# mspaintenjoyer/DepthEstimation

Hardware: AMD Instinct MI355X
Metric: disparity Mpix/s at 1080p d_max=128; 1/2/4/8-GPU scaling + %HBM roofline (higher is better)
Workload: dtype u8

## Files before the change

depthestimation_amd/csrc/dsx_api.hip:

```cpp
#include <hip/hip_runtime.h>

#include <cstdio>
#include <cstdlib>
#include <algorithm>
#include <cstring>
#include <string>
#include <vector>

#include "../../include/dsx.h"
#include "dsx_internal.h"

extern char **environ;

#ifndef DSX_RESET_LEFT
#define DSX_RESET_LEFT 1
#endif

namespace {

thread_local std::string g_err;

int fail(int code, const std::string &msg) {
    g_err = msg;
    return code;
// ... 365 lines not shown
        take("PRIO_T", e.prio_t);
        take("SLOW_W8", e.slow_w8);
        take("AGEW", e.agew);
        take("VARIANT", e.variant);
        take("TIMELINE", e.timeline);
    }
    return e;
}

dsx::Bm2Args base_args(dsx_handle *h, int H, int W, int64_t stride, const DsxEnv &env = dsx_env()) {
    dsx::Bm2Args a{};
    a.stride = stride;
    a.H = H;
    a.W = W;
    a.m = h->p.min_disp;
    a.D = h->p.num_disp;
    a.uniq = h->p.uniqueness_ratio;
    a.lr = h->p.disp12_max_diff;
    a.subpix = h->p.subpixel;
    a.float_mode = h->p.float_mode;
    a.padv = pad_value(h);
    a.strip_begin = 0;
    a.strip_count = (W + dsx::kStripWidth - 1) / dsx::kStripWidth;
    a.grid_override = h->p.grid_blocks;
    {
        const bool fl = h->p.in_flight != 0;
        a.prio = env.prio ? atoi(env.prio) : (fl ? 0 : 1);
        a.pt1 = 128, a.pt2 = 205, a.pt3 = 243;
        if (env.prio_t) sscanf(env.prio_t, "%d,%d,%d", &a.pt1, &a.pt2, &a.pt3);
        a.slow_w8 = env.slow_w8 ? atoi(env.slow_w8) : 11;
        a.agew[0] = fl ? 64 : 78, a.agew[1] = fl ? 64 : 70, a.agew[2] = a.agew[3] = 64;
        if (env.agew) sscanf(env.agew, "%d,%d,%d,%d", &a.agew[0], &a.agew[1], &a.agew[2], &a.agew[3]);
        a.nlev = 0;
        a.variant = env.variant ? atoi(env.variant) : 0;
    }
    a.nframes = 1;
    a.frame_stride = 0;
    return a;
}

#define DSX_LAUNCH(h, name, st, call)                                    \
    do {                                                                 \
        TimedLaunch t_;                                                  \
        if ((h)->p.timing) {                                             \
            int rc_ = begin_timed((h), (name), (st), t_);                \
            if (rc_) return rc_;                                         \
// ... 70 lines not shown
        a.ref = static_cast<const uint8_t *>(dL);
        a.src = static_cast<const uint8_t *>(dR);
        a.out_fixed = static_cast<int16_t *>(outFixed);
        a.out_float = static_cast<float *>(outFloat);
        a.nframes = nframes;
        a.frame_stride = frame_stride;
        if (lr) {
            a.side = dsx::SIDE_LEFT_LR;
            a.lr_keys = h->lrKeys + (size_t)h->lrParity * H * W * h->lrFrames;
            a.lr_reset = h->lrKeys + (size_t)(h->lrParity ^ 1) * H * W * h->lrFrames;
            a.lr_reset_n = DSX_RESET_LEFT ? (int64_t)H * W * h->lrDirty[h->lrParity ^ 1] : 0;
            a.dstar = h->dStar;
            a.kshift = h->g.kind != dsx::BM_SAD ? h->g.DB : 16;
        } else {
            if (lr_sg) {
                a.sg_keys = h->lrKeys + (size_t)h->lrParity * H * W * h->lrFrames;
                a.lr_reset = h->lrKeys + (size_t)(h->lrParity ^ 1) * H * W * h->lrFrames;
                a.lr_reset_n = (int64_t)H * W * h->lrDirty[h->lrParity ^ 1];
                a.dstar = h->dStar;
                a.kshift = h->g.kind != dsx::BM_SAD ? h->g.DB : 16;
            }
            const int xlo = std::max(0, h->p.min_disp + h->p.num_disp - 1);
            const int xhi = std::min(W - 1, W - 1 + h->p.min_disp);
            if (xlo > xhi) {
                a.strip_begin = 0;
                a.strip_count = 0;
            } else {
                a.strip_begin = xlo / dsx::kStripWidth;
                a.strip_count = xhi / dsx::kStripWidth + 1 - a.strip_begin;
            }
        }
        uint64_t *tl = nullptr;
        const char *tlpath = env.timeline;
        if (tlpath && *tlpath) DSX_HIP(hipMalloc(&tl, 12 * 8 * 65536));
        if (tl) DSX_HIP(hipMemsetAsync(tl, 0, 12 * 8 * 65536, st));
        a.timeline = tl;
        DSX_LAUNCH(h, "bm_pass_left", st, dsx::launch_bm2(radius, h->g.kind, h->g.NW, a, st));
        h->lastKeys = lr_sg ? a.sg_keys : (lr ? a.lr_keys : nullptr);
        h->lastDstar = h->dStar;
        h->lastKshift = a.kshift;
        if (lr_sg) {
            const int P = h->lrParity;
            if (!defer_lr)
                DSX_LAUNCH(h, "lr_fixup_sgbm", st,
                           dsx::launch_lr_fixup_sgbm(h->dStar, a.sg_keys, H * nframes, W, h->p.min_disp,
                                                     h->p.disp12_max_diff, a.kshift, a.out_fixed, a.out_float, st));
            h->lrDirty[P ^ 1] = 0;
            h->lrDirty[P] = nframes;
            h->lrParity = P ^ 1;
// ... 763 lines not shown
```

depthestimation_amd/csrc/dsx_bm.hip:

```cpp
#include "dsx_internal.h"
#include "dsx_partition.h"
#include "dsx_subpix.h"

constexpr int kWpe = 3;
constexpr int kWpeSsd = 4;

#ifndef DSX_ROWSTEP_PAIRTAIL
#define DSX_ROWSTEP_PAIRTAIL 0
#endif
#ifndef DSX_ROWSTEP_DIVQ
#define DSX_ROWSTEP_DIVQ 1
#endif
#ifndef DSX_ROWSTEP_OVERLAP
#define DSX_ROWSTEP_OVERLAP 1
#endif
#ifndef DSX_ROWSTEP_AHEAD
#define DSX_ROWSTEP_AHEAD 1
#endif
constexpr bool kRowstepOverlap = DSX_ROWSTEP_OVERLAP;
constexpr bool kRowstepAhead = DSX_ROWSTEP_AHEAD;
constexpr bool kRowstepPairtail = DSX_ROWSTEP_PAIRTAIL;
constexpr bool kRowstepDivq = DSX_ROWSTEP_DIVQ;
#ifndef DSX_ROWSTEP_ATID
#define DSX_ROWSTEP_ATID 1
#endif
#ifndef DSX_ROWSTEP_KEY2
#define DSX_ROWSTEP_KEY2 1
#endif
#ifndef DSX_ROWSTEP_MERGE
#define DSX_ROWSTEP_MERGE 1
#endif
constexpr bool kRowstepMerge = DSX_ROWSTEP_MERGE;
constexpr bool kRowstepAtid = DSX_ROWSTEP_ATID;
constexpr bool kRowstepKey2 = DSX_ROWSTEP_KEY2;

#include <algorithm>
#include <cstdio>
#include <cstdlib>
#include <cstring>
#include <mutex>
#include <type_traits>
#include <utility>
#include <vector>

namespace dsx {

typedef unsigned short u16x2 __attribute__((ext_vector_type(2)));
typedef uint32_t u32x2 __attribute__((ext_vector_type(2)));
__device__ __forceinline__ u32x2 lds_read_b64(const uint8_t *p) {
    return *(const volatile __attribute__((address_space(3))) u32x2 *)p;
}

__device__ __forceinline__ u16x2 as2(uint32_t v) { return __builtin_bit_cast(u16x2, v); }
__device__ __forceinline__ uint32_t as1(u16x2 v) { return __builtin_bit_cast(uint32_t, v); }
__device__ __forceinline__ int clampi2(int v, int lo, int hi) { return v < lo ? lo : (v > hi ? hi : v); }
__device__ __forceinline__ uint32_t umin2(uint32_t a, uint32_t b) { return a < b ? a : b; }
__device__ __forceinline__ u16x2 add_sub2(u16x2 a, u16x2 p, u16x2 q) { return as2(as1(a) + as1(p) - as1(q)); }
// ... 99 lines not shown
    return v;
}


typedef const __attribute__((address_space(4))) uint32_t cu32;
typedef const __attribute__((address_space(1))) uint8_t gu8;
typedef const __attribute__((address_space(1))) uint32_t gu32;
typedef __attribute__((address_space(1))) uint8_t gw8;
typedef __attribute__((address_space(1))) int16_t g16;
typedef __attribute__((address_space(1))) float gf32;

template <bool RELOAD>
__device__ __forceinline__ Bm2Args kargs_row(const Bm2Args &a) {
    if constexpr (RELOAD) {
        typedef __attribute__((address_space(4))) const Bm2Args KArgs;
        KArgs *p = (KArgs *)__builtin_amdgcn_kernarg_segment_ptr();
        asm volatile("" : "+s"(p));
        return *(const Bm2Args *)p;
    } else {
        return a;
    }
}

template <int R, bool SSD, int NW, int SIDE, bool FAST, bool ABS, bool LRFULL>
__device__ __forceinline__ void bm2_segment(const Bm2Args &a_in, uint8_t *smem, int x0, int yb, int ye, long fin, long fout,
                                            bool lr_on, int done0, const int (&pe)[3], int &qcur, int wvu
#ifdef DSX_STAMPS
                                            , uint64_t (&ph)[8], uint64_t &t_prev, uint64_t &nsteps
#endif
) {
    using G = Geo<R, SSD, NW>;
    constexpr int TX = G::TX, NC = G::NC, Dp = G::Dp, NT = G::NT, TPP = G::TPP, DSL = G::DSL, CB = G::CB,
                  PITCH = G::PITCH, NJ = G::NJ, SLOT = G::SLOT, NB = G::NB, NJ4 = (NJ + 3) / 4;
    constexpr int side = SIDE;
    const Bm2Args a = kargs_row<SIDE == 3>(a_in);
    constexpr bool FSS = SSD && !ABS && R <= 5 && (SIDE == 0 || SIDE == 3 || SIDE == 4);
    constexpr bool SGK = SIDE == 4;
    constexpr uint32_t OFF = FSS ? 0x4B000000u : 0u;
    constexpr int CW = (!FSS && (SSD || SIDE == 3)) ? 4 : 8, NCH = (NC + CW - 1) / CW;
    typedef typename std::conditional<FSS, float, typename std::conditional<SSD, uint32_t, u16x2>::type>::type acc_t;
    uint8_t *tile = smem + 4 * SLOT;

    constexpr bool LANE_RB = SSD && !ABS && NW >= 4;
    int ln = 0;
    if constexpr (LANE_RB)
        asm volatile("v_mbcnt_lo_u32_b32 %0, -1, 0\n\tv_mbcnt_hi_u32_b32 %0, -1, %0" : "=v"(ln));
    else
        ln = (int)threadIdx.x & 63;
    const int tid = LANE_RB ? (wvu << 6) + ln : (int)threadIdx.x;
    const int wv = LANE_RB ? wvu : tid >> 6;
    const int H = a.H, W = a.W, m = a.m, D = a.D;
    const int64_t stride = a.stride;
    const int d0 = SSD ? (wv * 64 + ln) : (wv * 128 + 2 * ln);
    const uint32_t padv = a.padv;
    const int PB = side == 1 ? (x0 - R + m) : (x0 - R - m + NC - 1);
    const int sgn = side == 1 ? 1 : -1;

    constexpr int NC4 = (NC + 3) / 4;
    constexpr bool RL2 = !SSD;
    uint32_t ofs_r = (uint32_t)(x0 - R + 4 * min(tid, NC4 - 1));
    uint32_t ofs_s = side == 1 ? (uint32_t)(PB + 4 * min(tid, NJ4 - 1)) : (uint32_t)(PB - 4 * min(tid, NJ4 - 1) - 3);
    constexpr bool MRG = kRowstepMerge && RL2 && FAST && SIDE != 3 && SIDE != 2 && !(SIDE == 4 && R >= 7);
    static_assert(!MRG || NJ4 + NC4 <= NT, "merged staging: a lane per staged dword");
    const bool m_s = tid < NJ4;
    const int m_r = min(tid - NJ4, NC4 - 1);
    const uint8_t *m_base = m_s ? a.src + fin + ofs_s : a.ref + fin + (uint32_t)(x0 - R + 4 * m_r);
    const bool m_dn = m_s && side != 1;
    const uint32_t m_sel0 = m_dn ? 0x0C0C0C03u : 0x0C0C0C00u, m_sel1 = m_dn ? 0x0C0C0C02u : 0x0C0C0C01u,
                   m_sel2 = m_dn ? 0x0C0C0C01u : 0x0C0C0C02u, m_sel3 = m_dn ? 0x0C0C0C00u : 0x0C0C0C03u;
    const uint32_t m_lane = m_s ? (uint32_t)(16 * tid) : (uint32_t)(G::SROW + 16 * m_r);
    auto ldm = [&](int r, uint32_t &w) __attribute__((always_inline)) {
        const int yy = clampi2(r, 0, H - 1);
        long ro = (long)yy * stride;
        asm("" : "+s"(ro));
        w = *reinterpret_cast<const uint32_t *>(m_base + ro);
    };
    auto stm = [&](uint8_t *sp, uint32_t w) __attribute__((always_inline)) {
        if (tid < NJ4 + NC4)
            *reinterpret_cast<uint4 *>(sp) = make_uint4(__builtin_amdgcn_perm(0u, w, m_sel0), __builtin_amdgcn_perm(0u, w, m_sel1),
                                                        __builtin_amdgcn_perm(0u, w, m_sel2), __builtin_amdgcn_perm(0u, w, m_sel3));
    };
    auto ld = [&](int r, uint32_t &w0, uint32_t &w1, uint32_t &w2, uint32_t &w3, uint32_t &rf) __attribute__((always_inline)) {
        const int yy = clampi2(r, 0, H - 1);
        const uint8_t *srow_ = a.src + fin + (long)yy * stride;
        const uint8_t *rrow_ = a.ref + fin + (long)yy * stride;
        if constexpr (RL2) {
            asm("" : "+s"(srow_));
            asm("" : "+s"(rrow_));
        }
        typedef typename std::conditional<RL2, gu8, const uint8_t>::type row8;
        typedef typename std::conditional<RL2, gu32, const uint32_t>::type row32;
        typedef typename std::conditional<RL2, uint32_t, int>::type rix;
// ... 128 lines not shown
    };
    auto pair_e0 = [](const uint32_t(&sw)[CW + 1], int c) __attribute__((always_inline)) -> uint32_t {
        return side == 1 ? sw[c] : sw[c + 1];
    };
    auto pair_e1 = [](const uint32_t(&sw)[CW + 1], int c) __attribute__((always_inline)) -> uint32_t {
        return side == 1 ? sw[c + 1] : sw[c];
    };

    acc_t cs[NC];
#pragma unroll
    for (int c = 0; c < NC; ++c) cs[c] = acc_t(0);
    constexpr bool SADINIT = ABS || R != 4 || SIDE != 3;
    if constexpr ((!SSD || ABS) && side != 1 && SADINIT) {
        constexpr int NGR = (2 * R + 1 + 3) / 4;
        constexpr int TPG = rnd16(NJ4 * 32);
        constexpr int RG = rnd16(NC4 * 16);
        static_assert(NGR * (TPG + RG) <= G::SMEM, "transposed init rows must fit the block's LDS");
        block_sync<NW>();
        auto ldb = [&](int r, uint32_t &w, uint32_t &e, uint32_t &rf) __attribute__((always_inline)) {
            const int yy = clampi2(r, 0, H - 1);
            const uint8_t *srow = a.src + fin + (long)yy * stride;
            const uint8_t *rrow = a.ref + fin + (long)yy * stride;
            const int tj = min(tid, NJ4 - 1), tr = min(tid, NC4 - 1);
            if constexpr (FAST) {
                const uint8_t *pp = srow + PB - 4 * tj - 3;
                w = *reinterpret_cast<const uint32_t *>(pp);
                e = pp[-1];
                rf = *reinterpret_cast<const uint32_t *>(rrow + x0 - R + 4 * tr);
            } else {
                uint32_t v = 0;
#pragma unroll
                for (int q = 0; q < 4; ++q) v |= (uint32_t)srow[clampi2(PB - 4 * tj - q, 0, W - 1)] << (8 * (3 - q));
                w = v;
                e = srow[clampi2(PB - 4 * tj - 4, 0, W - 1)];
                v = 0;
#pragma unroll
                for (int q = 0; q < 4; ++q) v |= (uint32_t)rrow[clampi2(x0 - R + 4 * tr + q, 0, W - 1)] << (8 * q);
                rf = v;
            }
        };
#pragma unroll 1
        for (int g = 0; g < NGR; ++g) {
            uint32_t w[4], e[4], rf[4];
#pragma unroll
            for (int r = 0; r < 4; ++r) {
                if (4 * g + r <= 2 * R) {
                    ldb(yb - R + 4 * g + r, w[r], e[r], rf[r]);
// ... 23 lines not shown
            }
            if (tid < NC4) {
                uint32_t Rv[4];
#pragma unroll
                for (int k = 0; k < 4; ++k) {
                    const uint32_t lo = __builtin_amdgcn_perm(rf[1], rf[0], 0x0C0C0000u | ((4u + k) << 8) | (uint32_t)k);
                    const uint32_t hi = __builtin_amdgcn_perm(rf[3], rf[2], 0x0C0C0000u | ((4u + k) << 8) | (uint32_t)k);
                    Rv[k] = __builtin_amdgcn_perm(hi, lo, 0x05040100u);
                }
                *reinterpret_cast<uint4 *>(smem + NGR * TPG + g * RG + 16 * tid) = make_uint4(Rv[0], Rv[1], Rv[2], Rv[3]);
            }
        }
        block_sync<NW>();
        const uint8_t *tb = smem + d0 * 8;
        {
        uint32_t ae[NC], ao[NC];
#pragma unroll
        for (int c = 0; c < NC; ++c) ae[c] = ao[c] = 0;
#pragma unroll 1
        for (int g = 0; g < NGR; ++g) {
#pragma unroll
            for (int q = 0; q < NC4; ++q) {
                const int c0 = 4 * q;
                const uint4 rr = *reinterpret_cast<const uint4 *>(smem + NGR * TPG + g * RG + 4 * c0);
                const uint32_t rv[4] = {rr.x, rr.y, rr.z, rr.w};
#pragma unroll
                for (int c = 0; c < 4; ++c) {
                    if (c0 + c < NC) {
                        if constexpr (ABS) {
                            const uint32_t p0 = *reinterpret_cast<const uint32_t *>(tb + g * TPG + (NC - 1 - c0 - c) * 8);
                            ae[c0 + c] = __builtin_amdgcn_sad_u8(rv[c], p0, ae[c0 + c]);
                        } else {
                            const uint2 pr = *reinterpret_cast<const uint2 *>(tb + g * TPG + (NC - 1 - c0 - c) * 8);
                            ae[c0 + c] = __builtin_amdgcn_sad_u8(rv[c], pr.x, ae[c0 + c]);
                            ao[c0 + c] = __builtin_amdgcn_sad_u8(rv[c], pr.y, ao[c0 + c]);
                        }
                    }
                }
            }
        }
#pragma unroll
        for (int c = 0; c < NC; ++c) {
            if constexpr (ABS) cs[c] = ae[c];
            else cs[c] = as2(ae[c] | (ao[c] << 16));
        }
        }
// ... 124 lines not shown
                for (int i = 0; i < 8; ++i) {
                    const bool hit = rel >= 8 * i - 1 && rel <= 8 * i + 8;
                    nm = hit ? nm : umin2(nm, emin8(*reinterpret_cast<const uint4 *>(epx + 16 * i)));
                }
                const int ib0 = (rel - 1) >> 3, ib1 = (rel + 1) >> 3;
#pragma unroll
                for (int t = 0; t < 2; ++t) {
                    const int ib = t == 0 ? ib0 : ib1;
                    if (ib >= 0 && ib < 8 && (t == 0 || ib1 != ib0)) {
                        const uint4 v = *reinterpret_cast<const uint4 *>(epx + 16 * ib);
                        const uint32_t c8[8] = {v.x & 0xFFFFu, v.x >> 16, v.y & 0xFFFFu, v.y >> 16,
                                                v.z & 0xFFFFu, v.z >> 16, v.w & 0xFFFFu, v.w >> 16};
#pragma unroll
                        for (int e = 0; e < 8; ++e) {
                            const int dd = 8 * ib + e - rel;
                            nm = (dd > 1 || dd < -1) ? umin2(nm, c8[e]) : nm;
                        }
                    }
                }
                nm = gmin<TPP>(nm);
                const uint32_t real_max = padv < (1u << 24) ? padv : (1u << 24);
                if (nm < real_max && nm * (uint32_t)(100 - a.uniq) < ecb * 100u) valid = false;
            }
            if (eh == 0 && ex < W) {
                const long o = fout + (long)ey * W + ex;
                const int16_t fx = valid ? (int16_t)(m * 16 + ef) : (int16_t)((m - 1) * 16);
                if (a.out_fixed) a.out_fixed[o] = fx;
                if (a.out_float) {
                    if (a.float_mode == 0) {
                        a.out_float[o] = (float)fx * 0.0625f;
                    } else {
                        float pf = (float)(m + eb);
                        if (esp) pf = (float)(m + eb) + (float)((int32_t)ecm - (int32_t)ecp) / (float)(2 * eden);
                        a.out_float[o] = valid ? pf : (float)(m - 1);
                    }
                }
            }
        }
    };
    for (int y = yb; y < ye; ++y) {
        const Bm2Args &a = kargs_row<SIDE == 3>(a_in);
#ifdef DSX_STAMPS
        ++nsteps;
#endif
        DSX_STAMP(0);
        if (a.prio) {
            const int dn = done0 + (y - yb);
// ... 64 lines not shown
                        sn[t][c + 1] = pn.x; sn[t][c] = pn.y; nxn = pn.x;
                        so[t][c + 1] = po.x; so[t][c] = po.y; nxo = po.x;
                    }
                }
            };
            auto sads = [&](auto qc) __attribute__((always_inline)) {
                constexpr int q = decltype(qc)::value, c0 = CQ * q, t = AHD ? (q & 1) : 0;
#pragma unroll
                for (int c = 0; c < CQ; ++c) {
                    if (c0 + c < NC) {
                        const uint32_t en = sad_hi_u8(rn[t][c], sn[t][c], __builtin_amdgcn_sad_u8(rn[t][c], sn[t][c + 1], as1(cs[c0 + c])));
                        const uint32_t lo = sad_hi_u8(ro[t][c], so[t][c], __builtin_amdgcn_sad_u8(ro[t][c], so[t][c + 1], 0u));
                        uint32_t v = en - lo;
                        if constexpr (OVL) asm volatile("" : "+v"(v));
                        cs[c0 + c] = as2(v);
                    }
                }
            };
            auto chunk = [&](auto qc) __attribute__((always_inline)) {
                constexpr int q = decltype(qc)::value;
                if constexpr (q < NQ) {
                    __builtin_amdgcn_sched_barrier(0);
                    if constexpr (OVL && q < NRS + 3) estage(qc, y - 1);
                    if constexpr (!AHD) rd(qc);
                    else if constexpr (q + 1 < NQ) rd(std::integral_constant<int, q + 1>{});
                    __builtin_amdgcn_sched_barrier(0);
                    sads(qc);
                }
            };
            if constexpr (AHD) rd(std::integral_constant<int, 0>{});
            chunk(std::integral_constant<int, 0>{}); chunk(std::integral_constant<int, 1>{});
            chunk(std::integral_constant<int, 2>{}); chunk(std::integral_constant<int, 3>{});
            chunk(std::integral_constant<int, 4>{}); chunk(std::integral_constant<int, 5>{});
            chunk(std::integral_constant<int, 6>{}); chunk(std::integral_constant<int, 7>{});
            chunk(std::integral_constant<int, 8>{}); chunk(std::integral_constant<int, 9>{});
            chunk(std::integral_constant<int, 10>{}); chunk(std::integral_constant<int, 11>{});
            static_assert(NQ <= 12 && NQ >= 7, "chunks of the overlapped column update");
            __builtin_amdgcn_sched_barrier(0);
            if constexpr (OVL) {
                if constexpr (NQ < NRS + 3) estage(std::integral_constant<int, NRS + 2>{}, y - 1);
                estage(std::integral_constant<int, NRS + 3>{}, y - 1);
            }
          }
        } else if (y > yb) {
            uint32_t nxn = 0, nxo = 0;
#pragma unroll
            for (int q = 0; q < NCH; ++q) {
                const int c0 = CW * q;
                uint32_t sn[CW + 1], so[CW + 1], rn[CW], ro[CW];
                ref_chunk(par, c0, rn);
                ref_chunk(par + 1, c0, ro);
                s_chunk(par, c0, sn, nxn);
                s_chunk(par + 1, c0, so, nxo);
#pragma unroll
                for (int c = 0; c < CW; ++c) {
                    if (c0 + c < NC) {
                        if constexpr (ABS) {
                            cs[c0 + c] = __builtin_amdgcn_sad_u16(rn[c], sn[c], cs[c0 + c]) -
                                         __builtin_amdgcn_sad_u16(ro[c], so[c], 0u);
                        } else if constexpr (SSD) {
                            const int tn = (int)rn[c] - (int)sn[c];
                            const int to = (int)ro[c] - (int)so[c];
                            const int nto = (int)so[c] - (int)ro[c];
                            cs[c0 + c] = (uint32_t)mad_i24(to, nto, mad_i24(tn, tn, (int)cs[c0 + c]));
                        } else {
                            const uint32_t en = sad_hi_u8(rn[c], pair_e1(sn, c), __builtin_amdgcn_sad_u8(rn[c], pair_e0(sn, c), as1(cs[c0 + c])));
                            const uint32_t lo = sad_hi_u8(ro[c], pair_e1(so, c), __builtin_amdgcn_sad_u8(ro[c], pair_e0(so, c), 0u));
                            cs[c0 + c] = as2(en - lo);
                        }
                    }
                }
// ... 96 lines not shown
                    const int xe = x0 + ln - m - dtop;
                    if (E != 0xFFFFFFFFu && xe >= 0 && xe < W) atomicMin(krow + xe, E);
                }
                const int xa = x0 + TX - 1 - m - d0;
                if (Ae != 0xFFFFFFFFu && xa >= 0 && xa < W) atomicMin(krow + xa, Ae);
                if constexpr (!SSD) {
                    if (Ao != 0xFFFFFFFFu && xa - 1 >= 0 && xa - 1 < W) atomicMin(krow + xa - 1, Ao);
                }
            } else if (ATID && lane_writes) {
                static_assert(!ATID || (TX % 8 == 0 && G::LDW * CB == 256), "addtid: a lane's tile bytes are 4 * lane");
                if constexpr (ATID) {
                const uint32_t mb = lds_offset(tile) + (uint32_t)wvu * (uint32_t)(G::LDW * CB);
                auto grp = [&](auto k0c) __attribute__((always_inline)) {
                    constexpr int k0 = decltype(k0c)::value;
                    uint32_t v[8];
#pragma unroll
                    for (int j = 0; j < 8; ++j) {
                        if (k0 + j > 0) acc = add_sub2(acc, cs[k0 + j + 2 * R], cs[k0 + j - 1]);
                        v[j] = as1(acc);
                    }
                    lds_store8_addtid<k0 * PITCH, PITCH>(mb, v);
                };
                grp(std::integral_constant<int, 0>{});
                grp(std::integral_constant<int, 8>{});
                grp(std::integral_constant<int, 16>{});
                grp(std::integral_constant<int, 24>{});
                }
            } else if (lane_writes) {
#pragma unroll
                for (int k = 0; k < TX; ++k) {
                    if (k > 0) {
                        if constexpr (FSS) acc = (acc - cs[k - 1]) + cs[k + 2 * R];
                        else if constexpr (SSD) acc = acc + cs[k + 2 * R] - cs[k - 1];
                        else acc = add_sub2(acc, cs[k + 2 * R], cs[k - 1]);
                    }
                    if constexpr (SSD) *reinterpret_cast<uint32_t *>(tb + k * PITCH) = abits(acc);
                    else *reinterpret_cast<uint32_t *>(tb + k * PITCH) = as1(acc);
                }
            }
            if (dodd && d0 + 1 == D) {
                for (int k = 0; k < TX; ++k) *reinterpret_cast<uint16_t *>(tb + k * PITCH + 2) = (uint16_t)padv;
            }
            if (edge && lane_writes) {
                const int base = x0 + m + d0;
                for (int k = 0; k < TX; ++k) {
                    const int p0 = base + k;
                    if constexpr (SSD) {
                        if (p0 < 0 || p0 > W - 1) *reinterpret_cast<uint32_t *>(tb + k * PITCH) = padv;
                    } else {
// ... 180 lines not shown
                    mp.x = pc[-1];
                    mp.y = pc[1];
                    const uint32_t c0 = (cb << 16) | ((uint32_t)valid << 15) | (uint32_t)b, c1 = as1(mp);
                    int sec = (y - yb) & 1;
                    asm("" : "+s"(sec));
                    const bool second = sec != 0;
                    if (second || !more) {
                        const bool prev = second && h == 0;
                        const uint32_t s0 = prev ? kp0 : c0, s1 = prev ? kp1 : c1;
                        const int tb = (int)(s0 & 0x7FFFu);
                        const int32_t tcb = (int32_t)(s0 >> 16), cm = (int32_t)(s1 & 0xFFFFu), cp = (int32_t)(s1 >> 16);
                        const bool tvalid = (s0 & 0x8000u) != 0;
                        int32_t f = tb * 16;
                        float pf = (float)(m + tb);
                        if (a.subpix) {
                            const bool sp = tb > 0 && tb < D - 1;
                            int32_t den = cm + cp - 2 * tcb;
                            den = den < 1 ? 1 : den;
                            const int32_t num = (cm - cp) * 16 + den;
                            const int32_t q = DIVQ ? subpix_quot(num, 2 * den) : div_trunc_small(num, 2 * den);
                            f += sp ? q : 0;
                            if (a.float_mode == 1 && sp) pf = (float)(m + tb) + (float)(cm - cp) / (float)(2 * den);
                        }
                        if ((second || h == 0) && x < W) {
                            long ro = fout + (long)(y - sec) * W;
                            asm("" : "+s"(ro));
                            const uint32_t xh = (uint32_t)(x + (h ? W : 0));
                            const int16_t fx = tvalid ? (int16_t)(m * 16 + f) : (int16_t)((m - 1) * 16);
                            if (a.out_fixed) {
                                int16_t *rowp = a.out_fixed + ro;
                                asm("" : "+s"(rowp));
                                *(g16 *)((gw8 *)rowp + 2u * xh) = fx;
                            }
                            if (a.out_float) {
                                float *rowp = a.out_float + ro;
                                asm("" : "+s"(rowp));
                                *(gf32 *)((gw8 *)rowp + 4u * xh) = a.float_mode == 0 ? (float)fx * 0.0625f : (tvalid ? pf : (float)(m - 1));
                            }
                        }
                    } else {
                        kp0 = c0;
                        kp1 = c1;
                    }
                } else {
                int32_t f = b * 16;
                float pf = (float)(m + b);
                if (a.subpix && b > 0 && b < D - 1) {
                    int32_t cm, cp;
                    const uint8_t *pk = tile + k * PITCH;
                    if constexpr (SSD) {
                        cm = (int32_t)(reinterpret_cast<const uint32_t *>(pk)[b - 1] - OFF);
                        cp = (int32_t)(reinterpret_cast<const uint32_t *>(pk)[b + 1] - OFF);
                    } else {
                        cm = reinterpret_cast<const uint16_t *>(pk)[b - 1];
                        cp = reinterpret_cast<const uint16_t *>(pk)[b + 1];
                    }
                    int32_t den = cm + cp - 2 * (int32_t)cb;
                    den = den < 1 ? 1 : den;
                    if constexpr (DIVQ) f += subpix_quot((cm - cp) * 16 + den, 2 * den);
                    else f += div_trunc_small((cm - cp) * 16 + den, 2 * den);
                    if (a.float_mode == 1) pf = (float)(m + b) + (float)(cm - cp) / (float)(2 * den);
                }
                if (h == 0 && x < W) {
                    if (lr_on) a.dstar[o] = valid ? (int16_t)b : (int16_t)-1;
                    const int16_t fx = valid ? (int16_t)(m * 16 + f) : (int16_t)((m - 1) * 16);
                    if constexpr (SGK) {
                        a.dstar[o] = fx;
                        if (valid)
                            atomicMin(a.sg_keys + fout + (long)y * W + (x - m - b),
                                      (cb << a.kshift) | (((1u << a.kshift) - 1u) - (uint32_t)b));
                    }
                    if (a.out_fixed) a.out_fixed[o] = fx;
                    if (a.out_float) a.out_float[o] = a.float_mode == 0 ? (float)fx * 0.0625f : (valid ? pf : (float)(m - 1));
                }
                }
            }
        }
        if (!RL2 && more) {
            st(par ^ 2, pn0, pn1, pn2, pn3, pnr);
            st((par ^ 2) + 1, po0, po1, po2, po3, por);
        }
        DSX_STAMP(6);
        block_sync<NW>();
        DSX_STAMP(7);
    }
    if constexpr (OVL) {
// ... 4 lines not shown
        dr(std::integral_constant<int, 3>{}); dr(std::integral_constant<int, 4>{}); dr(std::integral_constant<int, 5>{});
        dr(std::integral_constant<int, 6>{}); dr(std::integral_constant<int, 7>{}); dr(std::integral_constant<int, 8>{});
        dr(std::integral_constant<int, 9>{}); dr(std::integral_constant<int, 10>{}); dr(std::integral_constant<int, 11>{});
    }
}

template <int R, bool SSD, int NW, int SIDE, bool ABS>
__global__ __launch_bounds__(64 * NW) __attribute__((amdgpu_waves_per_eu((SSD && NW >= 4) ? kWpeSsd : kWpe))) void bm2(Bm2Args a) {
    using G = Geo<R, SSD, NW>;
    constexpr int TX = G::TX, NT = G::NT, NC = G::NC, NJ = G::NJ;
    constexpr int side = SIDE;
    extern __shared__ __attribute__((aligned(16))) uint8_t smem[];
    const int tid = threadIdx.x;
    const int wvu = __builtin_amdgcn_readfirstlane(tid >> 6);
    const int H = a.H, W = a.W, m = a.m;
    if (a.timeline && wvu == 0 && __lane_id() == 0) a.timeline[4 * blockIdx.x] = __builtin_amdgcn_s_memrealtime();
#ifdef DSX_STAMPS
    uint64_t ph[8] = {0, 0, 0, 0, 0, 0, 0, 0};
    uint64_t t_prev = 0;
    uint64_t nsteps = 0;
#endif

    if ((side == 0 || side == 3 || side == 4) && (a.out_fixed || a.out_float)) {
        const int xa = a.strip_begin * TX, xb = min(W, (a.strip_begin + a.strip_count) * TX);
        const int nin = xa + (W - xb);
        const int total = nin * H * a.nframes;
        const int16_t fi = (int16_t)((m - 1) * 16);
        for (int q = blockIdx.x * NT + tid; q < total; q += gridDim.x * NT) {
            const int y = q / nin;
            const int c = q - y * nin;
            const int x = c < xa ? c : xb + (c - xa);
            const long o = (long)y * W + x;
            if (a.out_fixed) a.out_fixed[o] = fi;
            if (a.out_float) a.out_float[o] = (float)(m - 1);
            if constexpr (side == 4) a.dstar[o] = fi;
        }
    }

    if ((side == 3 || side == 4) && a.lr_reset_n > 0) {
        uint32_t *kr = a.lr_reset;
        const int64_t n = a.lr_reset_n, stride = (int64_t)gridDim.x * NT;
        const int64_t t0 = (int64_t)blockIdx.x * NT + tid;
        if (((uintptr_t)kr & 15u) == 0) {
            for (int64_t q = t0; q < n / 4; q += stride)
                reinterpret_cast<uint4 *>(kr)[q] = make_uint4(0xFFFFFFFFu, 0xFFFFFFFFu, 0xFFFFFFFFu, 0xFFFFFFFFu);
            for (int64_t q = n / 4 * 4 + t0; q < n; q += stride) kr[q] = 0xFFFFFFFFu;
        } else {
            for (int64_t q = t0; q < n; q += stride) kr[q] = 0xFFFFFFFFu;
        }
    }

    const int lin0 = a.part[blockIdx.x], lin1 = a.part[blockIdx.x + 1];
    constexpr bool lr_on = SIDE == 3;
    int qcur = -1;
    int pe[3];
    {
        const int tot = lin1 - lin0;
        pe[0] = (a.pt1 * tot + 255) >> 8;
        pe[1] = (a.pt2 * tot + 255) >> 8;
        pe[2] = (a.pt3 * tot + 255) >> 8;
    }
    for (int it = lin0; it < lin1;) {
        const int sidx = it / H;
        const int f = sidx / a.strip_count;
        const int s = a.strip_begin + (sidx - f * a.strip_count);
        const long fin = (long)f * a.frame_stride, fout = (long)f * H * W;
        const int yb = it - sidx * H;
        const int ye = min(H, yb + (lin1 - it));
        const int done0 = it - lin0;
        it += ye - yb;
        const int x0 = s * TX;
        const int PB = side == 1 ? (x0 - R + m) : (x0 - R - m + NC - 1);
        const int NJ4 = (NJ + 3) / 4;
        const bool fast = (side == 1 ? (PB >= 0 && PB + 4 * NJ4 <= W - 1) : (PB - 4 * NJ4 >= 0 && PB <= W - 1)) &&
                          x0 - R >= 0 && x0 - R + 4 * ((NC + 3) / 4) - 1 <= W - 1;
#ifdef DSX_STAMPS
#define DSX_SEG(FASTV, FULLV) \
    bm2_segment<R, SSD, NW, SIDE, FASTV, ABS, FULLV>(a, smem, x0, yb, ye, fin, fout, lr_on, done0, pe, qcur, wvu, ph, t_prev, nsteps)
#else
#define DSX_SEG(FASTV, FULLV) bm2_segment<R, SSD, NW, SIDE, FASTV, ABS, FULLV>(a, smem, x0, yb, ye, fin, fout, lr_on, done0, pe, qcur, wvu)
#endif
        const bool lrfull = side == 3 && x0 + TX <= W && a.D == G::Dp;
        if (fast) {
            if (lrfull) DSX_SEG(true, true);
            else DSX_SEG(true, false);
        } else {
            if (lrfull) DSX_SEG(false, true);
            else DSX_SEG(false, false);
        }
#undef DSX_SEG
    }
    if (a.timeline && wvu == 0 && __lane_id() == 0) {
        const uint64_t t_end = __builtin_amdgcn_s_memrealtime();
        uint64_t *tl = a.timeline + 4 * blockIdx.x;
        tl[1] = t_end;
        tl[2] = (uint64_t)__builtin_amdgcn_s_getreg((4 << 0) | (0 << 6) | (31 << 11));
        tl[3] = (uint64_t)__builtin_amdgcn_s_getreg((20 << 0) | (0 << 6) | (15 << 11));
#ifdef DSX_STAMPS
        uint64_t *ps = a.timeline + 4 * 65536 + 8 * blockIdx.x;
        for (int i = 0; i < 7; ++i) ps[i] = ph[i];
        ps[7] = nsteps;
#endif
    }
}


struct PartKey {
    int dev, NG, S, sb, nframes, H, XL, XU, w8, nlev, w[4];
    bool operator==(const PartKey &o) const { return memcmp(this, &o, sizeof(PartKey)) == 0; }
};
static std::mutex &launch_mutex() {
    static std::mutex mu;
    return mu;
}
static hipError_t bm2_partition_dev(const PartKey &k, int TX, const int **out) {
    static std::vector<std::pair<PartKey, int *>> cache;
    for (const auto &e : cache)
        if (e.first == k) {
            *out = e.second;
            return hipSuccess;
        }
    if (cache.size() >= 256) {
        int prev = 0;
        (void)hipGetDevice(&prev);
        for (size_t i = 0; i < cache.size(); ++i) {
            bool seen = false;
            for (size_t j = 0; j < i; ++j) seen = seen || cache[j].first.dev == cache[i].first.dev;
            if (seen) continue;
            (void)hipSetDevice(cache[i].first.dev);
            hipError_t se = hipDeviceSynchronize();
            if (se != hipSuccess) {
                (void)hipSetDevice(prev);
                return se;
            }
        }
        for (auto &e : cache) {
            (void)hipSetDevice(e.first.dev);
            (void)hipFree(e.second);
        }
        (void)hipSetDevice(prev);
        cache.clear();
    }
    const std::vector<int> part = bm2_partition(k.NG, k.S, k.sb, k.nframes, k.H, k.XL, k.XU, TX, k.w8, k.nlev, k.w);
    int *d = nullptr;
    hipError_t e = hipMalloc(&d, part.size() * sizeof(int));
    if (e != hipSuccess) return e;
    e = hipMemcpy(d, part.data(), part.size() * sizeof(int), hipMemcpyHostToDevice);
    if (e != hipSuccess) {
        (void)hipFree(d);
        return e;
    }
    cache.emplace_back(k, d);
    *out = d;
    return hipSuccess;
}

template <int R, bool SSD, int NW, int SIDE, bool ABS = false>
static hipError_t launch_bm2_side(const Bm2Args &a, hipStream_t st) {
    using G = Geo<R, SSD, NW>;
    constexpr int SM = G::SMEM + ((SIDE == 3 && !SSD) ? G::XRB * NW : 0);
    const void *fn = (const void *)bm2<R, SSD, NW, SIDE, ABS>;
    static int blocks_per_cu[64] = {};
    static int num_cu[64] = {};
    int dev = 0;
    hipError_t e = hipGetDevice(&dev);
    if (e != hipSuccess) return e;
// ... 26 lines not shown
    static const bool verbose = getenv("DSX_VERBOSE") != nullptr;
    if (verbose)
        fprintf(stderr, "[dsx] bm2<R=%d,SSD=%d,NW=%d,SIDE=%d> grid %ld (%d/CU) smem %d\n", R, (int)SSD, NW, SIDE, grid,
                blocks_per_cu[dev], SM);
    Bm2Args la = a;
    la.nlev = 1;
    if (grid == (long)blocks_per_cu[dev] * num_cu[dev] && a.nframes == 1) {
        const int lv = blocks_per_cu[dev] * NW / 4;
        la.nlev = lv < 1 ? 1 : (lv > 4 ? 4 : lv);
    }
    {
        constexpr int NJ4 = (G::NJ + 3) / 4, NC4 = (G::NC + 3) / 4, NC = G::NC;
        const int W = a.W, m = a.m;
        PartKey k;
        memset(&k, 0, sizeof(k));
        k.dev = dev, k.NG = (int)grid, k.S = a.strip_count, k.sb = a.strip_begin, k.nframes = a.nframes, k.H = a.H;
        if (SIDE == 1) {
            k.XL = std::max(R - m, R);
            k.XU = std::min(W - 1 - 4 * NJ4 + R - m, W - 1 + R - 4 * NC4 + 1);
        } else {
            k.XL = std::max(4 * NJ4 + R + m - NC + 1, R);
            k.XU = std::min(W - 1 + R + m - NC + 1, W - 1 + R - 4 * NC4 + 1);
        }
        k.w8 = a.slow_w8, k.nlev = la.nlev;
        for (int i = 0; i < 4; ++i) k.w[i] = la.nlev > 1 ? a.agew[i] : 64;
        e = bm2_partition_dev(k, G::TX, &la.part);
        if (e != hipSuccess) return e;
    }
    hipLaunchKernelGGL((bm2<R, SSD, NW, SIDE, ABS>), dim3((unsigned)grid), dim3(G::NT), SM, st, la);
    return hipGetLastError();
}

template <int R, bool SSD, int NW>
static hipError_t launch_bm2_one(const Bm2Args &a, hipStream_t st) {
    switch (a.side) {
        case 0: return a.sg_keys ? launch_bm2_side<R, SSD, NW, 4>(a, st) : launch_bm2_side<R, SSD, NW, 0>(a, st);
        case 1: return launch_bm2_side<R, SSD, NW, 1>(a, st);
        case 3: return launch_bm2_side<R, SSD, NW, 3>(a, st);
        default: return launch_bm2_side<R, SSD, NW, 2>(a, st);
    }
}

template <int R>
static hipError_t launch_bm2_sad1(const Bm2Args &a, hipStream_t st) {
    switch (a.side) {
        case 0: return a.sg_keys ? launch_bm2_side<R, true, 1, 4, true>(a, st) : launch_bm2_side<R, true, 1, 0, true>(a, st);
        case 1: return launch_bm2_side<R, true, 1, 1, true>(a, st);
        case 3: return launch_bm2_side<R, true, 1, 3, true>(a, st);
// ... 52 lines not shown
```

depthestimation_amd/csrc/dsx_internal.h:

```cpp
#pragma once
#include <hip/hip_runtime.h>
#include <stdint.h>

namespace dsx {

enum Side : int { SIDE_LEFT = 0, SIDE_RIGHT = 1, SIDE_VOLUME = 2, SIDE_LEFT_LR = 3 };

constexpr int kVolThreads = 256;

struct Geometry {
    int NW, Dp, TX, TPP, DB;
    int kind;
};

struct Bm2Args {
    const uint8_t *ref;
    const uint8_t *src;
    int64_t stride;
    int nframes;
    int64_t frame_stride;
    int H, W;
    int m;
    int D;
    int side;
    int uniq, lr, subpix, float_mode;
    uint32_t padv;
    int strip_begin, strip_count;
    int grid_override;
    int prio;
    int pt1, pt2, pt3;
    int variant;
    int slow_w8;
    int agew[4];
    int nlev;
    const int *part;
    uint32_t *lr_keys;
    int kshift;
    int16_t *dstar;
    uint32_t *sg_keys;
    uint32_t *lr_reset;
    int64_t lr_reset_n;
    int16_t *out_fixed;
    float *out_float;
    int16_t *out_dR;
    void *vol;
    uint64_t *timeline;
};

struct VolArgs {
    const void *vol;
    int nsum;
    size_t sstride;
    int H, W, m, D, Dp, DB, TPP;
    int uniq, lr, subpix, float_mode;
    int lr_form;
    int16_t *out_fixed;
    float *out_float;
};

constexpr int kStripWidth = 32;

__device__ __forceinline__ int div_trunc_small(int num, int den2) {
    int q = (int)__builtin_truncf((float)num * __builtin_amdgcn_rcpf((float)den2));
    int r = num - q * den2;
    if (num >= 0) {
        if (r < 0) { --q; r += den2; }
        if (r >= den2) { ++q; }
    } else {
        if (r > 0) { ++q; r -= den2; }
// ... 144 lines not shown
```

depthestimation_amd/csrc/dsx_partition.h:

```cpp
#pragma once

#include <algorithm>
#include <vector>

namespace dsx {

inline std::vector<int> bm2_partition(int NG, int S, int sb, int nframes, int H, int XL, int XU, int TX, int slow_w8,
                                      int nlev, const int *agew) {
    std::vector<int> part(NG + 1);
    const int NS = S * nframes;
    if (NG < NS || NS <= 0) {
        const long T = (long)NS * H;
        for (int b = 0; b <= NG; ++b) part[b] = (int)(b * T / NG);
        return part;
    }
    auto fdiv = [](long x, long y) { return x >= 0 ? x / y : -((-x + y - 1) / y); };
    const int slo = std::min(std::max((int)fdiv(XL + TX - 1, TX) - sb, 0), S);
    const int shi = std::min(std::max((int)fdiv(XU, TX) - sb + 1, slo), S);
    int w8 = slow_w8;
    if (w8 < 8 || NG * 8 < NS * w8 + 8 * NS) w8 = 8;
    const int ex = w8 - 8;
    auto Pf = [&](int s) -> long { return 8L * s + (long)ex * (std::min(s, slo) + std::max(0, s - shi)); };
    const long Uf = Pf(S), U = Uf * nframes;
    auto P = [&](int g) -> long { const int f = g / S; return f * Uf + Pf(g - f * S); };
    int nl = nlev > 1 ? std::min(nlev, 4) : 1;
    {
        int wmin = 1 << 30, wmax = 0;
        for (int L = 0; L < nl; ++L) {
            wmin = std::min(wmin, agew[L]);
            wmax = std::max(wmax, agew[L]);
        }
        if (nl > 1 && (wmin < 1 || 8L * NG * wmin < U * wmax)) nl = 1;
    }
    std::vector<long> Q(NG + 1, 0);
    for (int b = 0; b < NG; ++b) Q[b + 1] = Q[b] + (nl > 1 ? agew[(long)b * nl / NG] : 64);
    const long Qtot = Q[NG];
    std::vector<int> start(NS + 1);
    int b = 0;
    for (int g = 0; g <= NS; ++g) {
        const long T = P(g) * Qtot;
        while (b < NG && Q[b] * U < T) ++b;
        start[g] = b;
    }
    for (int g = 0; g < NS; ++g) {
        const long q0 = Q[start[g]], qd = Q[start[g + 1]] - q0;
        for (int bb = start[g]; bb <= start[g + 1]; ++bb)
            part[bb] = g * H + (int)((Q[bb] - q0) * H / qd);
    }
    part[NG] = NS * H;
    return part;
}

}
```

Before: 44810.

## Clamp edge strips via byte selectors so all strips take the fast copy path

Edge strips used to fall back to a slower non-FAST staging path with a heavier partition weight (slow_w8). They now clamp load addresses and use byte-permute selectors to replicate edge pixels, so every strip in the SAD left passes takes the FAST path and the partition weights all strips equally. An optional ragged mode, off by default, trims compute and stores for partially valid edge strips and reweights the partition to match. The cost is extra perm/selector arithmetic on every load and added template complexity.

```diff
diff --git a/depthestimation_amd/csrc/dsx_api.hip b/depthestimation_amd/csrc/dsx_api.hip
--- a/depthestimation_amd/csrc/dsx_api.hip
+++ b/depthestimation_amd/csrc/dsx_api.hip
@@ -411,6 +411,8 @@
     a.padv = pad_value(h);
     a.strip_begin = 0;
     a.strip_count = (W + dsx::kStripWidth - 1) / dsx::kStripWidth;
+    a.xlo = 0;
+    a.xhi = W - 1;
     a.grid_override = h->p.grid_blocks;
     {
         const bool fl = h->p.in_flight != 0;
@@ -527,9 +529,13 @@
             }
             const int xlo = std::max(0, h->p.min_disp + h->p.num_disp - 1);
             const int xhi = std::min(W - 1, W - 1 + h->p.min_disp);
+            a.xlo = xlo;
+            a.xhi = xhi;
             if (xlo > xhi) {
                 a.strip_begin = 0;
                 a.strip_count = 0;
+                a.xlo = 0;
+                a.xhi = -1;
             } else {
                 a.strip_begin = xlo / dsx::kStripWidth;
                 a.strip_count = xhi / dsx::kStripWidth + 1 - a.strip_begin;
diff --git a/depthestimation_amd/csrc/dsx_bm.hip b/depthestimation_amd/csrc/dsx_bm.hip
--- a/depthestimation_amd/csrc/dsx_bm.hip
+++ b/depthestimation_amd/csrc/dsx_bm.hip
@@ -1,5 +1,6 @@
 #include "dsx_internal.h"
 #include "dsx_partition.h"
+#include "dsx_edgeclamp.h"
 #include "dsx_subpix.h"
 
 constexpr int kWpe = 3;
@@ -33,6 +34,22 @@
 constexpr bool kRowstepMerge = DSX_ROWSTEP_MERGE;
 constexpr bool kRowstepAtid = DSX_ROWSTEP_ATID;
 constexpr bool kRowstepKey2 = DSX_ROWSTEP_KEY2;
+#ifndef DSX_EDGE_SELCLAMP
+#define DSX_EDGE_SELCLAMP 1
+#endif
+constexpr bool kEdgeSelclamp = DSX_EDGE_SELCLAMP;
+template <int R, bool SSD, int SIDE>
+constexpr bool bm2_selclamp() {
+    return kEdgeSelclamp && kRowstepMerge && !SSD && (SIDE == 0 || (SIDE == 4 && R < 7));
+}
+#ifndef DSX_EDGE_RAGGED
+#define DSX_EDGE_RAGGED 0
+#endif
+constexpr bool kEdgeRagged = DSX_EDGE_RAGGED;
+template <int R, bool SSD, int SIDE>
+constexpr bool bm2_ragged() {
+    return kEdgeRagged && bm2_selclamp<R, SSD, SIDE>();
+}
 
 #include <algorithm>
 #include <cstdio>
@@ -178,8 +195,8 @@
     }
 }
 
-template <int R, bool SSD, int NW, int SIDE, bool FAST, bool ABS, bool LRFULL>
-__device__ __forceinline__ void bm2_segment(const Bm2Args &a_in, uint8_t *smem, int x0, int yb, int ye, long fin, long fout,
+template <int R, bool SSD, int NW, int SIDE, bool FAST, bool ABS, bool LRFULL, bool RAGGED = false>
+__device__ __forceinline__ void bm2_segment(const Bm2Args &a_in, uint8_t *smem, int x0, int ncols_in, int yb, int ye, long fin, long fout,
                                             bool lr_on, int done0, const int (&pe)[3], int &qcur, int wvu
 #ifdef DSX_STAMPS
                                             , uint64_t (&ph)[8], uint64_t &t_prev, uint64_t &nsteps
@@ -189,6 +206,9 @@
     constexpr int TX = G::TX, NC = G::NC, Dp = G::Dp, NT = G::NT, TPP = G::TPP, DSL = G::DSL, CB = G::CB,
                   PITCH = G::PITCH, NJ = G::NJ, SLOT = G::SLOT, NB = G::NB, NJ4 = (NJ + 3) / 4;
     constexpr int side = SIDE;
+    static_assert(!RAGGED || (!SSD && FAST && (SIDE == 0 || SIDE == 4)), "ragged form: pair layout, left passes, the one copy");
+    const int ncols = RAGGED ? __builtin_amdgcn_readfirstlane(ncols_in) : TX;
+    const int clim = ncols + 2 * R;
     const Bm2Args a = kargs_row<SIDE == 3>(a_in);
     constexpr bool FSS = SSD && !ABS && R <= 5 && (SIDE == 0 || SIDE == 3 || SIDE == 4);
     constexpr bool SGK = SIDE == 4;
@@ -218,12 +238,16 @@
     uint32_t ofs_s = side == 1 ? (uint32_t)(PB + 4 * min(tid, NJ4 - 1)) : (uint32_t)(PB - 4 * min(tid, NJ4 - 1) - 3);
     constexpr bool MRG = kRowstepMerge && RL2 && FAST && SIDE != 3 && SIDE != 2 && !(SIDE == 4 && R >= 7);
     static_assert(!MRG || NJ4 + NC4 <= NT, "merged staging: a lane per staged dword");
+    constexpr bool SELC = bm2_selclamp<R, SSD, SIDE>();
+    static_assert(!SELC || FAST, "selector clamp: every strip takes the FAST copy");
     const bool m_s = tid < NJ4;
     const int m_r = min(tid - NJ4, NC4 - 1);
-    const uint8_t *m_base = m_s ? a.src + fin + ofs_s : a.ref + fin + (uint32_t)(x0 - R + 4 * m_r);
+    const int m_p = m_s ? (int)ofs_s : x0 - R + 4 * m_r;
+    const uint8_t *m_base = (m_s ? a.src : a.ref) + fin + (uint32_t)(SELC ? edge_addr(m_p, W) : m_p);
     const bool m_dn = m_s && side != 1;
-    const uint32_t m_sel0 = m_dn ? 0x0C0C0C03u : 0x0C0C0C00u, m_sel1 = m_dn ? 0x0C0C0C02u : 0x0C0C0C01u,
-                   m_sel2 = m_dn ? 0x0C0C0C01u : 0x0C0C0C02u, m_sel3 = m_dn ? 0x0C0C0C00u : 0x0C0C0C03u;
+    const uint32_t m_s4 = SELC ? edge_sel4(m_p, W) : 0x03020100u;
+    const uint32_t m_sel0 = edge_word_sel(m_s4, m_dn ? 3 : 0), m_sel1 = edge_word_sel(m_s4, m_dn ? 2 : 1),
+                   m_sel2 = edge_word_sel(m_s4, m_dn ? 1 : 2), m_sel3 = edge_word_sel(m_s4, m_dn ? 0 : 3);
     const uint32_t m_lane = m_s ? (uint32_t)(16 * tid) : (uint32_t)(G::SROW + 16 * m_r);
     auto ldm = [&](int r, uint32_t &w) __attribute__((always_inline)) {
         const int yy = clampi2(r, 0, H - 1);
@@ -398,7 +422,12 @@
             const uint8_t *srow = a.src + fin + (long)yy * stride;
             const uint8_t *rrow = a.ref + fin + (long)yy * stride;
             const int tj = min(tid, NJ4 - 1), tr = min(tid, NC4 - 1);
-            if constexpr (FAST) {
+            if constexpr (SELC) {
+                const int ps = PB - 4 * tj - 3, pr = x0 - R + 4 * tr;
+                w = __builtin_amdgcn_perm(0u, *reinterpret_cast<const uint32_t *>(srow + edge_addr(ps, W)), edge_sel4(ps, W));
+                e = srow[clampi2(ps - 1, 0, W - 1)];
+                rf = __builtin_amdgcn_perm(0u, *reinterpret_cast<const uint32_t *>(rrow + edge_addr(pr, W)), edge_sel4(pr, W));
+            } else if constexpr (FAST) {
                 const uint8_t *pp = srow + PB - 4 * tj - 3;
                 w = *reinterpret_cast<const uint32_t *>(pp);
                 e = pp[-1];
@@ -468,6 +497,7 @@
 #pragma unroll
             for (int q = 0; q < NC4; ++q) {
                 const int c0 = 4 * q;
+                if (RAGGED && c0 >= clim) continue;
                 const uint4 rr = *reinterpret_cast<const uint4 *>(smem + NGR * TPG + g * RG + 4 * c0);
                 const uint32_t rv[4] = {rr.x, rr.y, rr.z, rr.w};
 #pragma unroll
@@ -638,7 +668,7 @@
                 const uint32_t real_max = padv < (1u << 24) ? padv : (1u << 24);
                 if (nm < real_max && nm * (uint32_t)(100 - a.uniq) < ecb * 100u) valid = false;
             }
-            if (eh == 0 && ex < W) {
+            if (eh == 0 && ex < W && (!RAGGED || ek < ncols)) {
                 const long o = fout + (long)ey * W + ex;
                 const int16_t fx = valid ? (int16_t)(m * 16 + ef) : (int16_t)((m - 1) * 16);
                 if (a.out_fixed) a.out_fixed[o] = fx;
@@ -749,10 +779,12 @@
                 if constexpr (q < NQ) {
                     __builtin_amdgcn_sched_barrier(0);
                     if constexpr (OVL && q < NRS + 3) estage(qc, y - 1);
-                    if constexpr (!AHD) rd(qc);
-                    else if constexpr (q + 1 < NQ) rd(std::integral_constant<int, q + 1>{});
-                    __builtin_amdgcn_sched_barrier(0);
-                    sads(qc);
+                    if (!RAGGED || CQ * q < clim) {
+                        if constexpr (!AHD) rd(qc);
+                        else if constexpr (q + 1 < NQ) rd(std::integral_constant<int, q + 1>{});
+                        __builtin_amdgcn_sched_barrier(0);
+                        sads(qc);
+                    }
                 }
             };
             if constexpr (AHD) rd(std::integral_constant<int, 0>{});
@@ -774,6 +806,7 @@
 #pragma unroll
             for (int q = 0; q < NCH; ++q) {
                 const int c0 = CW * q;
+                if (RAGGED && c0 >= clim) continue;
                 uint32_t sn[CW + 1], so[CW + 1], rn[CW], ro[CW];
                 ref_chunk(par, c0, rn);
                 ref_chunk(par + 1, c0, ro);
@@ -916,9 +949,9 @@
                     lds_store8_addtid<k0 * PITCH, PITCH>(mb, v);
                 };
                 grp(std::integral_constant<int, 0>{});
-                grp(std::integral_constant<int, 8>{});
-                grp(std::integral_constant<int, 16>{});
-                grp(std::integral_constant<int, 24>{});
+                if (!RAGGED || ncols > 8) grp(std::integral_constant<int, 8>{});
+                if (!RAGGED || ncols > 16) grp(std::integral_constant<int, 16>{});
+                if (!RAGGED || ncols > 24) grp(std::integral_constant<int, 24>{});
                 }
             } else if (lane_writes) {
 #pragma unroll
@@ -1145,7 +1178,7 @@
                             f += sp ? q : 0;
                             if (a.float_mode == 1 && sp) pf = (float)(m + tb) + (float)(cm - cp) / (float)(2 * den);
                         }
-                        if ((second || h == 0) && x < W) {
+                        if ((second || h == 0) && x < W && (!RAGGED || k < ncols)) {
                             long ro = fout + (long)(y - sec) * W;
                             asm("" : "+s"(ro));
                             const uint32_t xh = (uint32_t)(x + (h ? W : 0));
@@ -1184,7 +1217,7 @@
                     else f += div_trunc_small((cm - cp) * 16 + den, 2 * den);
                     if (a.float_mode == 1) pf = (float)(m + b) + (float)(cm - cp) / (float)(2 * den);
                 }
-                if (h == 0 && x < W) {
+                if (h == 0 && x < W && (!RAGGED || k < ncols)) {
                     if (lr_on) a.dstar[o] = valid ? (int16_t)b : (int16_t)-1;
                     const int16_t fx = valid ? (int16_t)(m * 16 + f) : (int16_t)((m - 1) * 16);
                     if constexpr (SGK) {
@@ -1235,7 +1268,8 @@
 #endif
 
     if ((side == 0 || side == 3 || side == 4) && (a.out_fixed || a.out_float)) {
-        const int xa = a.strip_begin * TX, xb = min(W, (a.strip_begin + a.strip_count) * TX);
+        constexpr bool RAGK = bm2_ragged<R, SSD, SIDE>();
+        const int xa = RAGK ? a.xlo : a.strip_begin * TX, xb = RAGK ? a.xhi + 1 : min(W, (a.strip_begin + a.strip_count) * TX);
         const int nin = xa + (W - xb);
         const int total = nin * H * a.nframes;
         const int16_t fi = (int16_t)((m - 1) * 16);
@@ -1282,25 +1316,36 @@
         const int ye = min(H, yb + (lin1 - it));
         const int done0 = it - lin0;
         it += ye - yb;
+        constexpr bool RAGK = bm2_ragged<R, SSD, SIDE>();
+        const int xr = RAGK ? max(s * TX, a.xlo) : s * TX;
+        const int ncols = RAGK ? min((s + 1) * TX, a.xhi + 1) - xr : TX;
         const int x0 = s * TX;
         const int PB = side == 1 ? (x0 - R + m) : (x0 - R - m + NC - 1);
         const int NJ4 = (NJ + 3) / 4;
         const bool fast = (side == 1 ? (PB >= 0 && PB + 4 * NJ4 <= W - 1) : (PB - 4 * NJ4 >= 0 && PB <= W - 1)) &&
                           x0 - R >= 0 && x0 - R + 4 * ((NC + 3) / 4) - 1 <= W - 1;
 #ifdef DSX_STAMPS
-#define DSX_SEG(FASTV, FULLV) \
-    bm2_segment<R, SSD, NW, SIDE, FASTV, ABS, FULLV>(a, smem, x0, yb, ye, fin, fout, lr_on, done0, pe, qcur, wvu, ph, t_prev, nsteps)
+#define DSX_SEGX(FASTV, FULLV, RAGV, X0V) \
+    bm2_segment<R, SSD, NW, SIDE, FASTV, ABS, FULLV, RAGV>(a, smem, X0V, ncols, yb, ye, fin, fout, lr_on, done0, pe, qcur, wvu, ph, t_prev, nsteps)
 #else
-#define DSX_SEG(FASTV, FULLV) bm2_segment<R, SSD, NW, SIDE, FASTV, ABS, FULLV>(a, smem, x0, yb, ye, fin, fout, lr_on, done0, pe, qcur, wvu)
+#define DSX_SEGX(FASTV, FULLV, RAGV, X0V) \
+    bm2_segment<R, SSD, NW, SIDE, FASTV, ABS, FULLV, RAGV>(a, smem, X0V, ncols, yb, ye, fin, fout, lr_on, done0, pe, qcur, wvu)
 #endif
+#define DSX_SEG(FASTV, FULLV) DSX_SEGX(FASTV, FULLV, false, s * TX)
         const bool lrfull = side == 3 && x0 + TX <= W && a.D == G::Dp;
-        if (fast) {
+        if constexpr (RAGK) {
+            if (ncols < TX) DSX_SEGX(true, false, true, xr);
+            else DSX_SEG(true, false);
+        } else if constexpr (bm2_selclamp<R, SSD, SIDE>()) {
+            DSX_SEG(true, false);
+        } else if (fast) {
             if (lrfull) DSX_SEG(true, true);
             else DSX_SEG(true, false);
         } else {
             if (lrfull) DSX_SEG(false, true);
             else DSX_SEG(false, false);
         }
+#undef DSX_SEGX
 #undef DSX_SEG
     }
     if (a.timeline && wvu == 0 && __lane_id() == 0) {
@@ -1319,7 +1364,7 @@
 
 
 struct PartKey {
-    int dev, NG, S, sb, nframes, H, XL, XU, w8, nlev, w[4];
+    int dev, NG, S, sb, nframes, H, XL, XU, w8, nlev, w[4], rw[2];
     bool operator==(const PartKey &o) const { return memcmp(this, &o, sizeof(PartKey)) == 0; }
 };
 static std::mutex &launch_mutex() {
@@ -1354,7 +1399,7 @@
         (void)hipSetDevice(prev);
         cache.clear();
     }
-    const std::vector<int> part = bm2_partition(k.NG, k.S, k.sb, k.nframes, k.H, k.XL, k.XU, TX, k.w8, k.nlev, k.w);
+    const std::vector<int> part = bm2_partition(k.NG, k.S, k.sb, k.nframes, k.H, k.XL, k.XU, TX, k.w8, k.nlev, k.w, k.rw[0], k.rw[1]);
     int *d = nullptr;
     hipError_t e = hipMalloc(&d, part.size() * sizeof(int));
     if (e != hipSuccess) return e;
@@ -1427,8 +1472,14 @@
             k.XL = std::max(4 * NJ4 + R + m - NC + 1, R);
             k.XU = std::min(W - 1 + R + m - NC + 1, W - 1 + R - 4 * NC4 + 1);
         }
-        k.w8 = a.slow_w8, k.nlev = la.nlev;
+        k.w8 = bm2_selclamp<R, SSD, SIDE>() ? 8 : a.slow_w8, k.nlev = la.nlev;
         for (int i = 0; i < 4; ++i) k.w[i] = la.nlev > 1 ? a.agew[i] : 64;
+        k.rw[0] = k.rw[1] = 8;
+        if (bm2_ragged<R, SSD, SIDE>() && a.strip_count > 0) {
+            const int s0 = a.strip_begin, s1 = a.strip_begin + a.strip_count - 1;
+            k.rw[0] = bm2_ragged_w8(std::min((s0 + 1) * G::TX, a.xhi + 1) - std::max(s0 * G::TX, a.xlo), R, G::TX);
+            if (s1 > s0) k.rw[1] = bm2_ragged_w8(std::min((s1 + 1) * G::TX, a.xhi + 1) - std::max(s1 * G::TX, a.xlo), R, G::TX);
+        }
         e = bm2_partition_dev(k, G::TX, &la.part);
         if (e != hipSuccess) return e;
     }
diff --git a/depthestimation_amd/csrc/dsx_edgeclamp.h b/depthestimation_amd/csrc/dsx_edgeclamp.h
--- /dev/null
+++ b/depthestimation_amd/csrc/dsx_edgeclamp.h
@@ -0,0 +1,26 @@
+#pragma once
+
+#include <cstdint>
+
+#if defined(__HIPCC__) || defined(__CUDACC__)
+#define DSX_EC_HD __host__ __device__ __forceinline__
+#else
+#define DSX_EC_HD inline
+#endif
+
+namespace dsx {
+
+DSX_EC_HD int edge_clampi(int v, int lo, int hi) { return v < lo ? lo : (v > hi ? hi : v); }
+
+DSX_EC_HD int edge_addr(int p, int W) { return edge_clampi(p, 0, W - 4); }
+
+DSX_EC_HD uint32_t edge_sel4(int p, int W) {
+    const int A = edge_addr(p, W);
+    uint32_t s = 0;
+    for (int k = 0; k < 4; ++k) s |= (uint32_t)(edge_clampi(p + k, 0, W - 1) - A) << (8 * k);
+    return s;
+}
+
+DSX_EC_HD uint32_t edge_word_sel(uint32_t sel4, int k) { return 0x0C0C0C00u | ((sel4 >> (8 * k)) & 0xFFu); }
+
+}
diff --git a/depthestimation_amd/csrc/dsx_internal.h b/depthestimation_amd/csrc/dsx_internal.h
--- a/depthestimation_amd/csrc/dsx_internal.h
+++ b/depthestimation_amd/csrc/dsx_internal.h
@@ -45,6 +45,7 @@
     int16_t *out_dR;
     void *vol;
     uint64_t *timeline;
+    int xlo, xhi;
 };
 
 struct VolArgs {
diff --git a/depthestimation_amd/csrc/dsx_partition.h b/depthestimation_amd/csrc/dsx_partition.h
--- a/depthestimation_amd/csrc/dsx_partition.h
+++ b/depthestimation_amd/csrc/dsx_partition.h
@@ -5,8 +5,15 @@
 
 namespace dsx {
 
+inline int bm2_ragged_w8(int ncols, int R, int TX) {
+    if (ncols >= TX) return 8;
+    const int upd = std::min(TX + 2 * R, (std::max(ncols, 1) + 2 * R + 3) / 4 * 4);
+    const int w = 3 + (5 * upd + (TX + 2 * R) / 2) / (TX + 2 * R);
+    return std::min(std::max(w, 1), 8);
+}
+
 inline std::vector<int> bm2_partition(int NG, int S, int sb, int nframes, int H, int XL, int XU, int TX, int slow_w8,
-                                      int nlev, const int *agew) {
+                                      int nlev, const int *agew, int rag_first_w8 = 8, int rag_last_w8 = 8) {
     std::vector<int> part(NG + 1);
     const int NS = S * nframes;
     if (NG < NS || NS <= 0) {
@@ -20,9 +27,23 @@
     int w8 = slow_w8;
     if (w8 < 8 || NG * 8 < NS * w8 + 8 * NS) w8 = 8;
     const int ex = w8 - 8;
-    auto Pf = [&](int s) -> long { return 8L * s + (long)ex * (std::min(s, slo) + std::max(0, s - shi)); };
-    const long Uf = Pf(S), U = Uf * nframes;
-    auto P = [&](int g) -> long { const int f = g / S; return f * Uf + Pf(g - f * S); };
+    std::vector<long> Pf(S + 1, 0);
+    int wsmin = 8;
+    auto fill = [&](bool ragged) {
+        wsmin = 8;
+        for (int s = 0; s < S; ++s) {
+            int w = 8 + ((s < slo || s >= shi) ? ex : 0);
+            if (ragged && s == S - 1 && rag_last_w8 != 8) w = rag_last_w8;
+            if (ragged && s == 0 && rag_first_w8 != 8) w = S == 1 ? std::min(rag_first_w8, w) : rag_first_w8;
+            wsmin = std::min(wsmin, w);
+            Pf[s + 1] = Pf[s] + w;
+        }
+    };
+    const bool rag = (rag_first_w8 != 8 || rag_last_w8 != 8) && rag_first_w8 >= 1 && rag_last_w8 >= 1;
+    fill(rag);
+    if (rag && (long)wsmin * NG < Pf[S] * nframes) fill(false);
+    const long Uf = Pf[S], U = Uf * nframes;
+    auto P = [&](int g) -> long { const int f = g / S; return f * Uf + Pf[g - f * S]; };
     int nl = nlev > 1 ? std::min(nlev, 4) : 1;
     {
         int wmin = 1 << 30, wmax = 0;
@@ -30,7 +51,7 @@
             wmin = std::min(wmin, agew[L]);
             wmax = std::max(wmax, agew[L]);
         }
-        if (nl > 1 && (wmin < 1 || 8L * NG * wmin < U * wmax)) nl = 1;
+        if (nl > 1 && (wmin < 1 || (long)wsmin * NG * wmin < U * wmax)) nl = 1;
     }
     std::vector<long> Q(NG + 1, 0);
     for (int b = 0; b < NG; ++b) Q[b + 1] = Q[b] + (nl > 1 ? agew[(long)b * nl / NG] : 64);
```

Measured after the change: 44700. No clear change (-0.2%).
